# url-kaist/Quatro

Measured on NVIDIA H100. Metric: registrations/sec (64-ring pair), higher is better.
Workload: dtype f32 (front end, match, graph filter) / f64 (graph boundary, GNC, COTE)

## Files before the change

include/quatro_b200.h:

```cpp
#ifndef QUATRO_B200_H_
#define QUATRO_B200_H_

#include <stdint.h>

#ifdef __cplusplus
extern "C" {
#endif

#define QB200_VERSION 100

typedef enum qb200_status {
  QB200_OK = 0,
  QB200_DEGENERATE_CLIQUE = 1,
  QB200_DEGENERATE_INPUT = 2,
  QB200_CAPACITY_EXCEEDED = 3,
  QB200_ERR_BAD_ARG = -1,
  QB200_ERR_NO_DEVICE = -2,
  QB200_ERR_CUDA = -3,
  QB200_ERR_UNSUPPORTED = -4,
  QB200_ERR_VOXEL_OVERFLOW = -5
} qb200_status;

enum { QB200_FLAG_CLIQUE_TRUNCATED = 1  };
#define QB200_DEFAULT_CLIQUE_NODE_LIMIT 262144
// ... 154 lines not shown
                                const qb200_params* p, qb200_result* res);

int qb200_match_and_pack(qb200_handle* h, const float* src4, int32_t n_src, const float* tgt4,
                         int32_t n_tgt, const qb200_params* p, int32_t* corr, float* src_matched4,
                         float* tgt_matched4, int32_t cap, int32_t* n_corr);

typedef struct qb200_corr_set {
  const float* a;
  const float* b;
  int32_t L;
  int32_t reserved;
} qb200_corr_set;
int qb200_solve_batch(qb200_handle* h, const qb200_corr_set* sets, int32_t n_sets, const qb200_params* p,
                      qb200_mem_kind kind, qb200_result* results);

typedef struct qb200_pair_lists {
  int32_t cap_per_pair;
  int32_t kind;
  int32_t* corr;
  float* src_matched4;
  float* tgt_matched4;
  int32_t* clique;
  int32_t* final_inliers;
  uint8_t* rot_inlier_mask;
  uint8_t* trans_inlier_mask;
} qb200_pair_lists;
enum { QB200_FLAG_LISTS_TRUNCATED = 2  };

int qb200_solve_batch_ex(qb200_handle* h, const qb200_corr_set* sets, int32_t n_sets, const qb200_params* p, qb200_mem_kind kind,
                         qb200_result* results, const qb200_pair_lists* lists);

int qb200_register_batch_enqueue(qb200_handle* h, const qb200_pair* pairs, int32_t n_pairs, const qb200_params* p, qb200_mem_kind kind,
                                 qb200_result* results);
int qb200_register_batch_flush(qb200_handle* h);
int qb200_register_batch_enqueue_ex(qb200_handle* h, const qb200_pair* pairs, int32_t n_pairs, const qb200_params* p,
                                    qb200_mem_kind kind, qb200_result* results, const qb200_pair_lists* lists);

int qb200_register_pair(qb200_handle* h, const float* src4, int32_t n_src, const float* tgt4,
                        int32_t n_tgt, const qb200_params* p, qb200_result* res);

int qb200_register_batch(qb200_handle* h, const qb200_pair* pairs, int32_t n_pairs,
                         const qb200_params* p, qb200_mem_kind kind, qb200_result* results);
int qb200_register_batch_ex(qb200_handle* h, const qb200_pair* pairs, int32_t n_pairs, const qb200_params* p, qb200_mem_kind kind,
                            qb200_result* results, const qb200_pair_lists* lists);

typedef struct qb200_slot_pair { int32_t src_slot, tgt_slot; } qb200_slot_pair;
int qb200_cache_reserve(qb200_handle* h, int32_t n_slots);
int qb200_cache_scans(qb200_handle* h, const float* const* scans4, const int32_t* n_points, const int32_t* slot_ids, int32_t n_scans,
                      const qb200_params* p, qb200_mem_kind kind);
int qb200_register_cached(qb200_handle* h, const qb200_slot_pair* pairs, int32_t n_pairs, const qb200_params* p, qb200_result* results);
int qb200_register_cached_ex(qb200_handle* h, const qb200_slot_pair* pairs, int32_t n_pairs, const qb200_params* p,
                             qb200_result* results, const qb200_pair_lists* lists);
int qb200_cache_copy(qb200_handle* h, int32_t from_slot, int32_t to_slot);
int qb200_cache_read(qb200_handle* h, int32_t slot, float* vox4, float* normals4, float* desc33, int32_t cap, int32_t* n);

#define QB200_UNIQUE_ID_BYTES 128
int qb200_comm_init_all(qb200_handle** handles, int32_t n_dev);
int qb200_register_batch_sharded(qb200_handle** handles, int32_t n_dev, const qb200_pair* pairs, int32_t n_pairs,
                                 const qb200_params* p, qb200_mem_kind kind, qb200_result* results);
int qb200_comm_unique_id(void* id128);
int qb200_comm_init_rank(qb200_handle* h, int32_t world, int32_t rank, const void* id128);
int qb200_register_batch_rank(qb200_handle* h, const qb200_pair* local_pairs, int32_t n_local, const qb200_params* p,
                              qb200_mem_kind kind, qb200_result* all_results, int32_t defer);
int qb200_comm_wait(qb200_handle* h);
int qb200_bind_numa(qb200_handle* h);

int qb200_get_last_clique(qb200_handle* h, int32_t* idx, int32_t cap, int32_t* n);
int qb200_get_last_final_inliers(qb200_handle* h, int32_t* idx, int32_t cap, int32_t* n);
int qb200_get_last_correspondences(qb200_handle* h, int32_t* corr, float* src_matched4,
                                   float* tgt_matched4, int32_t cap, int32_t* n);

int qb200_get_last_features(qb200_handle* h, int32_t which, float* normals4, float* desc33, int32_t cap, int32_t* n);

int qb200_get_stage_ms(qb200_handle* h, float* ms, int32_t n);

int qb200_get_kernel_ms(qb200_handle* h, float* ms, int32_t* launches, int32_t n);

int qb200_debug_tc_distances(qb200_handle* h, const float* a33, int32_t na, const float* b33, int32_t nb, float* out);


int qb200_debug_match_stats(qb200_handle* h, uint64_t* out4, int32_t reset);
int qb200_debug_nn_tables(qb200_handle* h, uint64_t* rowbest, int32_t cap_rows, uint64_t* colbest, int32_t cap_cols);
int qb200_debug_tc_profile(qb200_handle* h, uint64_t* out24, int32_t reset);
int qb200_debug_tc_footprint(qb200_handle* h, int32_t* out5);

int qb200_debug_match_verify(qb200_handle* h, uint64_t* out2, int32_t reset);

#ifdef __cplusplus
}
#endif
#endif
```

quatro_b200/capi.py:

```python
from __future__ import annotations

import ctypes as C
from typing import Optional, Sequence

import numpy as np

from . import _build

PMC_EXACT, PMC_HEU, KCORE_HEU, INLIER_NONE = 0, 1, 2, 3
FLAG_CLIQUE_TRUNCATED = 1
FLAG_LISTS_TRUNCATED = 2
COTE_MEDIAN, COTE_WEIGHTED_MEAN = 0, 1
MEM_HOST, MEM_DEVICE = 0, 1

STATUS_NAMES = {0: "OK", 1: "DEGENERATE_CLIQUE", 2: "DEGENERATE_INPUT", 3: "CAPACITY_EXCEEDED", -1: "ERR_BAD_ARG",
                -2: "ERR_NO_DEVICE", -3: "ERR_CUDA", -4: "ERR_UNSUPPORTED", -5: "ERR_VOXEL_OVERFLOW"}


class Params(C.Structure):
    _fields_ = [
        ("voxel_size", C.c_float), ("normal_radius", C.c_float), ("fpfh_radius", C.c_float), ("grid_cell", C.c_float),
        ("tuple_scale", C.c_float), ("use_crosscheck", C.c_int32), ("use_tuple_test", C.c_int32),
        ("tuple_trials_per_corr", C.c_int32), ("skip_flagged", C.c_int32), ("reserved0", C.c_int32),
        ("seed", C.c_uint64),
# ... 98 lines not shown

    def trimmed(self, records: np.ndarray) -> list:
        out = []
        for i, r in enumerate(records):
            d = {}
            for name, a in self.arrays.items():
                m = 0 if r["status"] == 3 else min(int(r[LIST_LAYOUT[name][2]]), self.cap)
                d[name] = a[i, :m].copy() if self.kind == MEM_HOST else a[i, :m]
            out.append(d)
        return out


RESULT_DTYPE = np.dtype([
    ("valid", "<i4"), ("status", "<i4"), ("n_src_vox", "<i4"), ("n_tgt_vox", "<i4"), ("n_mutual", "<i4"),
    ("n_corr", "<i4"), ("max_core", "<i4"), ("clique_size", "<i4"), ("gnc_iters", "<i4"), ("n_rot_inliers", "<i4"),
    ("n_final_inliers", "<i4"), ("flags", "<i4"), ("n_edges", "<i8"), ("cost", "<f8"), ("T", "<f8", (16,)),
])
assert RESULT_DTYPE.itemsize == C.sizeof(Result)


class QuatroB200Error(RuntimeError):
    def __init__(self, code: int, where: str, detail: str = ""):
        self.code = code
        super().__init__(f"{where}: {STATUS_NAMES.get(code, code)} {detail}")


_LIB: Optional[C.CDLL] = None


def _f32(a, cols=None) -> np.ndarray:
    a = np.ascontiguousarray(a, dtype=np.float32)
    if cols is not None:
        assert a.ndim == 2 and a.shape[1] == cols, (a.shape, cols)
    return a


def _ptr(a: Optional[np.ndarray]):
    return None if a is None else a.ctypes.data_as(C.c_void_p)


def load_library(build: bool = True) -> C.CDLL:
    global _LIB
    if _LIB is not None:
        return _LIB
    path = _build.build_cuda() if build else _build.CUDA_LIB
    lib = C.CDLL(str(path))
    vp, i32, i64, f32, f64 = C.c_void_p, C.c_int32, C.c_int64, C.c_float, C.c_double
    P = C.POINTER
    sig = {
        "qb200_default_params": (None, [P(Params)]),
        "qb200_default_config": (None, [P(Config)]),
        "qb200_version": (i32, []),
        "qb200_create": (i32, [P(Config), P(vp)]),
        "qb200_destroy": (None, [vp]),
        "qb200_set_stream": (i32, [vp, vp]),
        "qb200_last_error": (C.c_char_p, [vp]),
        "qb200_launch_count": (i64, [vp]),
        "qb200_voxelize": (i32, [vp, vp, i32, f32, i32, vp, i32, P(i32)]),
        "qb200_default_patchwork_params": (None, [P(PatchworkParams)]),
        "qb200_default_segment_params": (None, [P(SegmentParams)]),
        "qb200_segment_cloud": (i32, [vp, vp, i32, P(SegmentParams), vp, P(i32), vp, P(i32)]),
        "qb200_patchwork": (i32, [vp, vp, i32, P(PatchworkParams), vp, P(i32), vp, P(i32)]),
        "qb200_compute_fpfh": (i32, [vp, vp, i32, f32, f32, f32, vp, vp]),
        "qb200_match": (i32, [vp, vp, i32, vp, vp, i32, vp, P(Params), vp, i32, P(i32), P(i32)]),
        "qb200_build_graph": (i32, [vp, vp, vp, i32, f64, f64, vp, i32, vp, P(i64)]),
        "qb200_max_clique": (i32, [vp, vp, i32, i32, i32, f64, vp, P(i32), vp, vp, P(i32)]),
        "qb200_max_clique_ex": (i32, [vp, vp, i32, i32, i32, f64, i64, vp, P(i32), vp, vp, P(i32), P(i32)]),
        "qb200_solve_pose": (i32, [vp, vp, vp, i32, vp, i32, P(Params), P(Result), vp, vp]),
        "qb200_solve_correspondences": (i32, [vp, vp, vp, i32, P(Params), P(Result)]),
        "qb200_match_and_pack": (i32, [vp, vp, i32, vp, i32, P(Params), vp, vp, vp, i32, P(i32)]),
        "qb200_register_pair": (i32, [vp, vp, i32, vp, i32, P(Params), P(Result)]),
        "qb200_register_batch": (i32, [vp, P(Pair), i32, P(Params), i32, vp]),
        "qb200_get_last_clique": (i32, [vp, vp, i32, P(i32)]),
        "qb200_get_last_final_inliers": (i32, [vp, vp, i32, P(i32)]),
        "qb200_get_last_correspondences": (i32, [vp, vp, vp, vp, i32, P(i32)]),
        "qb200_get_stage_ms": (i32, [vp, vp, i32]),
        "qb200_get_kernel_ms": (i32, [vp, vp, vp, i32]),
        "qb200_debug_tc_distances": (i32, [vp, vp, i32, vp, i32, vp]),
        "qb200_debug_match_stats": (i32, [vp, vp, i32]),
        "qb200_debug_nn_tables": (i32, [vp, vp, i32, vp, i32]),
        "qb200_register_batch_enqueue": (i32, [vp, vp, i32, vp, i32, vp]),
        "qb200_register_batch_flush": (i32, [vp]),
        "qb200_debug_tc_profile": (i32, [vp, vp, i32]),
        "qb200_debug_tc_footprint": (i32, [vp, vp]),
        "qb200_solve_batch": (i32, [vp, vp, i32, vp, i32, vp]),
        "qb200_comm_init_all": (i32, [P(vp), i32]),
        "qb200_register_batch_sharded": (i32, [P(vp), i32, P(Pair), i32, P(Params), i32, vp]),
        "qb200_comm_unique_id": (i32, [vp]),
        "qb200_comm_init_rank": (i32, [vp, i32, i32, vp]),
        "qb200_register_batch_rank": (i32, [vp, P(Pair), i32, P(Params), i32, vp, i32]),
        "qb200_comm_wait": (i32, [vp]),
        "qb200_bind_numa": (i32, [vp]),
        "qb200_debug_match_verify": (i32, [vp, vp, i32]),
        "qb200_get_last_features": (i32, [vp, i32, vp, vp, i32, P(i32)]),
        "qb200_cache_reserve": (i32, [vp, i32]),
        "qb200_cache_scans": (i32, [vp, P(vp), P(i32), P(i32), i32, P(Params), i32]),
        "qb200_register_cached": (i32, [vp, vp, i32, P(Params), vp]),
        "qb200_cache_copy": (i32, [vp, i32, i32]),
        "qb200_cache_read": (i32, [vp, i32, vp, vp, vp, i32, P(i32)]),
        "qb200_register_batch_ex": (i32, [vp, vp, i32, P(Params), i32, vp, P(PairLists)]),
        "qb200_register_batch_enqueue_ex": (i32, [vp, vp, i32, P(Params), i32, vp, P(PairLists)]),
        "qb200_register_cached_ex": (i32, [vp, vp, i32, P(Params), vp, P(PairLists)]),
        "qb200_solve_batch_ex": (i32, [vp, vp, i32, P(Params), i32, vp, P(PairLists)]),
    }
    for name, (res, args) in sig.items():
        fn = getattr(lib, name)
        fn.restype = res
        fn.argtypes = args
    _LIB = lib
    return lib


EXPORTED_SYMBOLS = [
    "qb200_default_params", "qb200_default_config", "qb200_version", "qb200_create", "qb200_destroy",
    "qb200_set_stream", "qb200_last_error", "qb200_launch_count", "qb200_voxelize", "qb200_compute_fpfh",
    "qb200_default_patchwork_params", "qb200_patchwork", "qb200_default_segment_params", "qb200_segment_cloud", "qb200_match", "qb200_build_graph", "qb200_max_clique", "qb200_max_clique_ex", "qb200_solve_pose", "qb200_solve_correspondences",
    "qb200_match_and_pack", "qb200_register_pair", "qb200_register_batch", "qb200_get_last_clique",
    "qb200_get_last_final_inliers", "qb200_get_last_correspondences", "qb200_get_stage_ms", "qb200_get_kernel_ms",
    "qb200_debug_tc_distances",
    "qb200_debug_match_stats",
    "qb200_debug_nn_tables",
    "qb200_register_batch_enqueue",
    "qb200_register_batch_flush",
    "qb200_debug_tc_profile",
    "qb200_debug_tc_footprint",
    "qb200_solve_batch",
    "qb200_comm_init_all", "qb200_register_batch_sharded", "qb200_comm_unique_id", "qb200_comm_init_rank",
    "qb200_register_batch_rank", "qb200_comm_wait", "qb200_bind_numa",
    "qb200_debug_match_verify", "qb200_get_last_features", "qb200_cache_reserve", "qb200_cache_scans", "qb200_register_cached", "qb200_cache_copy", "qb200_cache_read",
    "qb200_register_batch_ex", "qb200_register_batch_enqueue_ex", "qb200_register_cached_ex", "qb200_solve_batch_ex",
]


def default_params() -> Params:
    p = Params()
    p.voxel_size, p.normal_radius, p.fpfh_radius, p.grid_cell = 0.3, 0.5, 0.75, 0.0
    p.tuple_scale, p.use_crosscheck, p.use_tuple_test, p.tuple_trials_per_corr = 0.95, 1, 1, 100
    p.skip_flagged, p.seed = 1, 0x5EED
    p.noise_bound, p.cbar2, p.rot_noise_bound, p.cote_noise_bound = 0.3, 1.0, 0.0, 0.3
    p.rotation_gnc_factor, p.rotation_cost_threshold, p.kcore_heuristic_threshold = 1.4, 0.00011, 0.5
    p.rotation_max_iterations, p.inlier_selection_mode, p.cote_mode = 50, PMC_HEU, COTE_MEDIAN
    p.using_rot_inliers_when_estimating_cote, p.use_pre_estimated_RyRx = 0, 0
    for i in range(9):
        p.RyRx[i] = 1.0 if i in (0, 4, 8) else 0.0
    return p


def comm_init_all(handles: Sequence["Handle"]):
    arr = (C.c_void_p * len(handles))(*[h.h for h in handles])
    st = load_library().qb200_comm_init_all(arr, len(handles))
    if st != 0:
        raise QuatroB200Error(st, "qb200_comm_init_all")


def register_batch_sharded(handles: Sequence["Handle"], pairs: Sequence, params: "Params", kind: int = 0) -> np.ndarray:
    n = len(pairs)
    arr = (Pair * n)()
    keep = []
    for i, pr in enumerate(pairs):
        if kind == MEM_HOST:
            s, t = _f32(pr[0], 4), _f32(pr[1], 4)
            keep.append((s, t))
            arr[i].src, arr[i].n_src, arr[i].tgt, arr[i].n_tgt = s.ctypes.data, len(s), t.ctypes.data, len(t)
        else:
            arr[i].src, arr[i].n_src, arr[i].tgt, arr[i].n_tgt = pr[0], pr[1], pr[2], pr[3]
    out = np.zeros(n, RESULT_DTYPE)
    hs = (C.c_void_p * len(handles))(*[h.h for h in handles])
    st = load_library().qb200_register_batch_sharded(hs, len(handles), arr, n, C.byref(params), kind, _ptr(out))
    if st != 0:
        raise QuatroB200Error(st, "qb200_register_batch_sharded " + handles[0].last_error())
    return out


def default_patchwork_params() -> PatchworkParams:
    p = PatchworkParams()
    load_library().qb200_default_patchwork_params(C.byref(p))
    return p


def default_segment_params() -> SegmentParams:
    p = SegmentParams()
    load_library().qb200_default_segment_params(C.byref(p))
    return p


def default_config() -> Config:
    c = Config()
    c.device, c.max_batch_slots, c.max_raw_points, c.max_voxel_points, c.max_corr = 0, 64, 131072, 16384, 4096
    return c


class Handle:

    def __init__(self, config: Optional[Config] = None, **kw):
        self.lib = load_library()
        cfg = config or default_config()
        for k, v in kw.items():
            setattr(cfg, k, v)
        self.cfg = cfg
        h = C.c_void_p()
        st = self.lib.qb200_create(C.byref(cfg), C.byref(h))
        if st != 0:
            raise QuatroB200Error(st, "qb200_create")
        self.h = h

    def close(self):
        if getattr(self, "h", None):
# ... 237 lines not shown
        out = np.zeros(len(sp), RESULT_DTYPE)
        self._check(self.lib.qb200_register_cached(self.h, _ptr(sp), len(sp), C.byref(params), _ptr(out)), "qb200_register_cached")
        return out

    def cache_copy(self, from_slot: int, to_slot: int):
        self._check(self.lib.qb200_cache_copy(self.h, from_slot, to_slot), "qb200_cache_copy")

    def cache_read(self, slot: int, cap: Optional[int] = None):
        cap = cap or self.cfg.max_voxel_points
        vox, nrm, desc = np.zeros((cap, 4), np.float32), np.zeros((cap, 4), np.float32), np.zeros((cap, 33), np.float32)
        n = C.c_int32(0)
        self._check(self.lib.qb200_cache_read(self.h, slot, _ptr(vox), _ptr(nrm), _ptr(desc), cap, C.byref(n)), "qb200_cache_read")
        m = min(n.value, cap)
        return vox[:m].copy(), nrm[:m].copy(), desc[:m].copy()

    @staticmethod
    def comm_unique_id() -> bytes:
        buf = C.create_string_buffer(128)
        st = load_library().qb200_comm_unique_id(buf)
        if st != 0:
            raise QuatroB200Error(st, "qb200_comm_unique_id")
        return buf.raw

    def comm_init_rank(self, world: int, rank: int, unique_id: bytes):
        buf = C.create_string_buffer(unique_id, 128)
        self._check(self.lib.qb200_comm_init_rank(self.h, world, rank, buf), "qb200_comm_init_rank")
        self.world, self.rank = world, rank

    def register_batch_rank_raw(self, pair_array, n_local: int, params: Params, kind: int, out_all: np.ndarray, defer: bool = False):
        return self._check(self.lib.qb200_register_batch_rank(self.h, pair_array, n_local, C.byref(params), kind, _ptr(out_all), int(defer)),
                           "qb200_register_batch_rank")

    def bind_numa(self) -> int:
        return int(self.lib.qb200_bind_numa(self.h))

    def comm_wait(self):
        return self._check(self.lib.qb200_comm_wait(self.h), "qb200_comm_wait")

    def register_batch_raw(self, pair_array, n: int, params: Params, kind: int, out: np.ndarray):
        return self._check(self.lib.qb200_register_batch(self.h, pair_array, n, C.byref(params), kind, _ptr(out)), "qb200_register_batch")

    def register_batch_enqueue_raw(self, pair_array, n: int, params: Params, kind: int, out: np.ndarray):
        return self._check(self.lib.qb200_register_batch_enqueue(self.h, pair_array, n, C.byref(params), kind, _ptr(out)), "qb200_register_batch_enqueue")

    def register_batch_flush(self):
        return self._check(self.lib.qb200_register_batch_flush(self.h), "qb200_register_batch_flush")

    def last_clique(self, cap: int = 1 << 16):
        idx = np.zeros(cap, np.int32)
        n = C.c_int32(0)
        self._check(self.lib.qb200_get_last_clique(self.h, _ptr(idx), cap, C.byref(n)), "qb200_get_last_clique")
        return idx[: n.value].copy()

    def last_final_inliers(self, cap: int = 1 << 16):
        idx = np.zeros(cap, np.int32)
        n = C.c_int32(0)
        self._check(self.lib.qb200_get_last_final_inliers(self.h, _ptr(idx), cap, C.byref(n)), "qb200_get_last_final_inliers")
        return idx[: n.value].copy()

    def last_correspondences(self, cap: int = 1 << 16):
        corr = np.zeros((cap, 2), np.int32)
        sm = np.zeros((cap, 4), np.float32)
        tm = np.zeros((cap, 4), np.float32)
        n = C.c_int32(0)
        self._check(self.lib.qb200_get_last_correspondences(self.h, _ptr(corr), _ptr(sm), _ptr(tm), cap, C.byref(n)),
                    "qb200_get_last_correspondences")
        return corr[: n.value].copy(), sm[: n.value].copy(), tm[: n.value].copy()

    def debug_match_stats(self, reset: bool = True) -> dict:
        out = np.zeros(4, np.uint64)
        self._check(self.lib.qb200_debug_match_stats(self.h, _ptr(out), int(reset)), "qb200_debug_match_stats")
        return {"exact_evals": int(out[0]), "tiles": int(out[1]), "warmups": int(out[2]), "aborted_stripes": int(out[3])}

    def debug_nn_tables(self, n_src: int, n_tgt: int):
        rb, cb = np.full(n_src, ~np.uint64(0)), np.full(n_tgt, ~np.uint64(0))
        self._check(self.lib.qb200_debug_nn_tables(self.h, _ptr(rb), n_src, _ptr(cb), n_tgt), "qb200_debug_nn_tables")
        return rb, cb

    def debug_tc_profile(self, reset: bool = True) -> np.ndarray:
        out = np.zeros(24, np.uint64)
        self._check(self.lib.qb200_debug_tc_profile(self.h, _ptr(out), int(reset)), "qb200_debug_tc_profile")
        return out

    def debug_tc_footprint(self) -> dict:
        out = np.zeros(5, np.int32)
        self._check(self.lib.qb200_debug_tc_footprint(self.h, _ptr(out)), "qb200_debug_tc_footprint")
        return {"threads": int(out[0]), "dyn_smem": int(out[1]), "static_smem": int(out[2]), "regs": int(out[3]),
                "ctas_per_sm": int(out[4])}

    def debug_match_verify(self, reset: bool = True) -> dict:
        out = np.zeros(2, np.uint64)
        self._check(self.lib.qb200_debug_match_verify(self.h, _ptr(out), int(reset)), "qb200_debug_match_verify")
        return {"compared": int(out[0]), "mismatches": int(out[1])}

    def debug_tc_distances(self, a33, b33) -> np.ndarray:
        a33, b33 = _f32(a33, 33), _f32(b33, 33)
        out = np.zeros((128, 128), np.float32)
        self._check(self.lib.qb200_debug_tc_distances(self.h, _ptr(a33), len(a33), _ptr(b33), len(b33), _ptr(out)), "qb200_debug_tc_distances")
        return out[: len(a33), : len(b33)].copy()

    def kernel_ms(self):
        ms = np.zeros(2, np.float32)
        calls = np.zeros(2, np.int32)
        self.lib.qb200_get_kernel_ms(self.h, _ptr(ms), _ptr(calls), 2)
        return ms, calls

    def stage_ms(self) -> np.ndarray:
        ms = np.zeros(8, np.float32)
        self.lib.qb200_get_stage_ms(self.h, _ptr(ms), 8)
        return ms
```

quatro_b200/csrc/clique.cu:

```cuda
#include "handle.cuh"

namespace qb {

__device__ __forceinline__ int warp_max(int v) { return __reduce_max_sync(0xffffffffu, v); }
__device__ __forceinline__ int warp_sum(int v) { return __reduce_add_sync(0xffffffffu, v); }

__device__ void warp_bucket_sort(const unsigned short* __restrict__ key, int n, int maxkey, int* __restrict__ bin,
                                 unsigned short* __restrict__ pos, unsigned short* __restrict__ vert) {
  const int lane = lane_id();
  for (int d = lane; d <= maxkey + 1; d += 32) bin[d] = 0;
  __syncwarp();
  for (int v = lane; v < n; v += 32) atomicAdd(&bin[key[v]], 1);
  __syncwarp();
  int carry = 0;
  for (int base = 0; base <= maxkey + 1; base += 32) {
    const int d = base + lane;
    const int c = d <= maxkey + 1 ? bin[d] : 0;
    int tot;
    const int ex = warp_excl_scan(c, &tot);
    if (d <= maxkey + 1) bin[d] = carry + ex;
    carry += tot;
  }
  __syncwarp();
  for (int base = 0; base < n; base += 32) {
    const int v = base + lane;
    const bool act = v < n;
    const int d = act ? key[v] : -1 - lane;
    const unsigned peers = __match_any_sync(0xffffffffu, d);
    const int rank = __popc(peers & ((1u << lane) - 1));
    const int b = act ? bin[d] : 0;
    __syncwarp();
    if (act) {
      pos[v] = (unsigned short)(b + rank);
      vert[b + rank] = (unsigned short)v;
      if (rank == 0) bin[d] = b + __popc(peers);
    }
    __syncwarp();
  }
  for (int base = ((maxkey + 1) / 32) * 32; base >= 0; base -= 32) {
    const int d = base + lane;
    int prev = 0;
    if (d >= 1 && d <= maxkey + 1) prev = bin[d - 1];
    __syncwarp();
    if (d >= 1 && d <= maxkey + 1) bin[d] = prev;
    __syncwarp();
  }
  if (lane == 0) bin[0] = 0;
  __syncwarp();
}

constexpr int kRing = 16;

__device__ __forceinline__ void cp_async4(void* smem_dst, const void* gsrc) {
  const unsigned d = (unsigned)__cvta_generic_to_shared(smem_dst);
  asm volatile("cp.async.ca.shared.global [%0], [%1], 4;" ::"r"(d), "l"(gsrc) : "memory");
}
__device__ __forceinline__ void cp_async_commit() { asm volatile("cp.async.commit_group;" ::: "memory"); }
template <int N>
__device__ __forceinline__ void cp_async_wait() { asm volatile("cp.async.wait_group %0;" ::"n"(N) : "memory"); }

constexpr int kKcWarps = 4;

__device__ __forceinline__ void kcore_apply_moves(const unsigned short* __restrict__ nbl, int cnt, int dv, int* __restrict__ bin,
                                                  unsigned short* __restrict__ deg, unsigned short* __restrict__ pos,
                                                  unsigned short* __restrict__ vert, unsigned short* __restrict__ mrk,
                                                  uint32_t* __restrict__ above_own, uint32_t* __restrict__ add_next, bool classes) {
  const int lane = lane_id();
  const unsigned lt = (1u << lane) - 1u;
  for (int c0 = 0; c0 < cnt; c0 += 32) {
    const int e = c0 + lane;
    const bool act = e < cnt;
    const int u = act ? nbl[e] : 0;
    const int du = act ? deg[u] : -1 - lane;
    const unsigned grp = __match_any_sync(0xffffffffu, du);
    const int rank = __popc(grp & lt), m = __popc(grp);
    int b0 = 0, pu = 0;
    if (act) {
      b0 = bin[du];
      pu = pos[u];
      mrk[u] = (unsigned short)(rank + 1);
    }
    __syncwarp();
    int y = -1;
    if (act && pu >= b0 + m) {
      int curk = rank;
      for (;;) {
        y = vert[b0 + curk];
        const int r = mrk[y];
        if (r == 0) break;
        curk = r - 1;
      }
    }
    __syncwarp();
    if (act) {
      vert[b0 + rank] = (unsigned short)u; pos[u] = (unsigned short)(b0 + rank);
      if (y >= 0) { vert[pu] = (unsigned short)y; pos[y] = (unsigned short)pu; }
      mrk[u] = 0;
      deg[u] = (unsigned short)(du - 1);
      const uint32_t bit = 1u << (u & 31);
      if (classes) {
        atomicAnd(&above_own[u >> 5], ~bit);
        if (du - 1 > dv) atomicOr(&add_next[u >> 5], bit);
      } else if (du - 1 == dv) {
        atomicAnd(&above_own[u >> 5], ~bit);
      }
      if (rank == 0) bin[du] = b0 + m;
    }
    __syncwarp();
  }
}

template <int WPL>
__device__ __forceinline__ int kcore_expand(const uint32_t (&w)[WPL], int w0, unsigned short* __restrict__ nbl) {
  int c = 0;
#pragma unroll
  for (int k = 0; k < WPL; ++k) c += __popc(w[k]);
  int cnt;
  int off = warp_excl_scan(c, &cnt);
  if (cnt != 0) {
#pragma unroll
    for (int k = 0; k < WPL; ++k) {
      uint32_t x = w[k];
      const int basebit = (w0 + k) * 32;
      while (x) {
        const int b = __ffs(x) - 1;
        x &= x - 1;
        nbl[off++] = (unsigned short)(basebit + b);
      }
    }
  }
  return cnt;
}

template <int WPL, bool kWs>
__global__ void __maxnreg__(168) kcore_kernel(const uint32_t* __restrict__ adj, const int* __restrict__ deg_in,
                                                              const int* __restrict__ n_corr, int Lc, int W, int Ls, int row_words,
                                                              unsigned char* __restrict__ ws, int* __restrict__ kcore,
                                                              int* __restrict__ korder, int* __restrict__ rank_of, int* __restrict__ by_rank,
                                                              int* __restrict__ kbin, int* __restrict__ max_core_out) {
  constexpr int NW = kKcWarps, AW = 32 * WPL;
  extern __shared__ __align__(16) unsigned char smem_raw[];
  __shared__ int ring_tag[kRing];

  const int pair = blockIdx.x, tid = threadIdx.x, lane = tid & 31, warp = tid >> 5;
  const int L = n_corr[pair];
  if ((L > Ls) != kWs) return;
  constexpr bool in_smem = !kWs;
  const int Lv = in_smem ? Ls : Lc;
  int* bin = in_smem ? reinterpret_cast<int*>(smem_raw)
                     : reinterpret_cast<int*>(ws + (size_t)pair * kcore_ws_bytes(Lc));
  uint32_t* above = in_smem ? reinterpret_cast<uint32_t*>(bin + Ls + 2)
                            : reinterpret_cast<uint32_t*>(smem_raw);
  uint32_t* add = above + NW * AW;
  uint32_t* rows = add + 2 * NW * AW;
  unsigned short* deg = in_smem ? reinterpret_cast<unsigned short*>(rows + row_words) : reinterpret_cast<unsigned short*>(bin + Lc + 2);
  unsigned short* pos = deg + Lv;
  unsigned short* vert = pos + Lv;
  unsigned short* mrk = vert + Lv;
  unsigned short* nbl_all = mrk + Lv;
  int* __restrict__ kc = kcore + (size_t)pair * (Lc + 2);
  int* __restrict__ ko = korder + (size_t)pair * (Lc + 2);
  int* __restrict__ ro = rank_of + (size_t)pair * (Lc + 2);
  int* __restrict__ br = by_rank + (size_t)pair * (Lc + 2);
  int* __restrict__ kb = kbin + (size_t)pair * (Lc + 2);
  if (L <= 0) {
    if (tid == 0) max_core_out[pair] = 0;
    return;
  }
  const uint32_t* __restrict__ G = adj + (size_t)pair * Lc * W;
  const int nbw = (L + 31) >> 5;
  const int nwl = (nbw + 31) >> 5;
  const bool cached = in_smem && (long long)L * nbw <= (long long)row_words;
  const int rs = in_smem ? Ls / 32 : W;
  const int w0 = lane * nwl;
  unsigned short* nbl = nbl_all + (size_t)warp * Lv;

  int md = 0;
  for (int v = tid; v < L; v += NW * 32) {
    const int d = deg_in[(size_t)pair * Lc + v];
    deg[v] = (unsigned short)d;
    mrk[v] = 0;
    md = max(md, d);
  }
  if (cached)
    for (int idx = tid; idx < L * nbw; idx += NW * 32) rows[idx] = G[(size_t)(idx / nbw) * W + (idx % nbw)];
  for (int wd = tid; wd < 3 * NW * AW; wd += NW * 32) above[wd] = 0u;
  __shared__ int s_md[NW];
  md = warp_max(md);
  if (lane == 0) s_md[warp] = md;
  __syncthreads();
  md = max(max(s_md[0], s_md[1]), max(s_md[2], s_md[3]));
  if (warp == 0) warp_bucket_sort(deg, L, md, bin, pos, vert);
  __syncthreads();
  for (int v = tid; v < L; v += NW * 32) {
    const int c = cached ? 0 : (int)deg[v] % NW;
    atomicOr(&above[c * AW + (v >> 5)], 1u << (v & 31));
  }
  __syncthreads();

  int cur = -1;
  if (cached) {
    if (warp != 0) return;
    for (int i = 0; i < L; ++i) {
      const int v = vert[i];
      const int dv = deg[v];
      if (dv > cur) {
        const int end = bin[dv + 1];
        for (int p = i + lane; p < end; p += 32) {
          const int x = vert[p];
          atomicAnd(&above[x >> 5], ~(1u << (x & 31)));
        }
        cur = dv;
        __syncwarp();
      }
      uint32_t w[WPL];
#pragma unroll
      for (int k = 0; k < WPL; ++k) w[k] = (k < nwl && w0 + k < nbw) ? (rows[v * nbw + w0 + k] & above[w0 + k]) : 0u;
      const int cnt = kcore_expand<WPL>(w, w0, nbl);
      if (cnt == 0) continue;
      __syncwarp();
      kcore_apply_moves(nbl, cnt, dv, bin, deg, pos, vert, mrk, above, above, false);
    }
  } else {
    uint32_t* above_w = above + warp * AW;
    const int lower = (warp + NW - 1) % NW;
    auto fetch = [&](int p) {
      if (p < L) {
        const int x = vert[p], sl = p % kRing;
        if (lane == 0) ring_tag[sl] = x;
#pragma unroll
        for (int k = 0; k < WPL; ++k)
          if (k < nwl && w0 + k < nbw) cp_async4(rows + sl * rs + w0 + k, G + (size_t)x * W + w0 + k);
      }
      cp_async_commit();
    };
    if (warp == 0) {
      for (int p = 0; p < kRing - 1; ++p) fetch(p);
      cp_async_wait<kRing - 2>();
    }
    __syncthreads();
    for (int i = 0; i < L; ++i) {
      const int v = vert[i];
      const int dv = deg[v];
      const int par = i & 1;
      if (warp == 0) fetch(i + kRing - 1);
      uint32_t* add_in = add + ((par ^ 1) * NW + warp) * AW;
      uint32_t w[WPL];
      const int sl = i % kRing;
      const bool hit = ring_tag[sl] == v;
#pragma unroll
      for (int k = 0; k < WPL; ++k) {
        w[k] = 0u;
        if (k < nwl && w0 + k < nbw) {
          const uint32_t a = add_in[w0 + k];
          if (a) { above_w[w0 + k] |= a; add_in[w0 + k] = 0u; }
          w[k] = hit ? rows[sl * rs + w0 + k] : G[(size_t)v * W + w0 + k];
        }
      }
      __syncwarp();
      if (dv > cur) {
        if (dv % NW == warp) {
          const int end = bin[dv + 1];
          for (int p = i + lane; p < end; p += 32) {
            const int x = vert[p];
            atomicAnd(&above_w[x >> 5], ~(1u << (x & 31)));
          }
          __syncwarp();
        }
        cur = dv;
      }
#pragma unroll
      for (int k = 0; k < WPL; ++k) w[k] = (k < nwl && w0 + k < nbw) ? (w[k] & above_w[w0 + k]) : 0u;
      const int cnt = kcore_expand<WPL>(w, w0, nbl);
      if (cnt != 0) {
        __syncwarp();
        kcore_apply_moves(nbl, cnt, dv, bin, deg, pos, vert, mrk, above_w, add + (par * NW + lower) * AW, true);
      }
      if (warp == 0) cp_async_wait<kRing - 2>();
      __syncthreads();
    }
    if (warp == 0) cp_async_wait<0>();
    if (warp != 0) return;
  }
  __syncwarp();
  const int max_core = deg[vert[L - 1]];
  for (int v = lane; v < L; v += 32) {
    kc[v] = (int)deg[v] + 1;
    ko[v] = vert[v];
  }
  if (lane == 0) max_core_out[pair] = max_core;
  __syncwarp();
  warp_bucket_sort(deg, L, max_core, bin, pos, vert);
  for (int v = lane; v < L; v += 32) {
    ro[v] = pos[v];
    br[v] = vert[v];
  }
  for (int d = lane; d <= max_core + 1; d += 32) kb[d] = bin[d];
}

__global__ void __launch_bounds__(256) permute_adj_kernel(const uint32_t* __restrict__ adj, const int* __restrict__ n_corr, int Lc, int W,
                                                          const int* __restrict__ rank_of, uint32_t* __restrict__ adjp) {
  extern __shared__ uint32_t rows[];
  const int pair = blockIdx.y;
  const int L = n_corr[pair];
  const int wib = threadIdx.x >> 5, lane = lane_id();
// ... 280 lines not shown
    const int begin = lb[depth];
    const uint32_t e = LP[begin + n_here - 1];
    __syncwarp();
    if (lane == 0) ln[depth] = n_here - 1;
    const int v = (int)(e & 0xFFFFu), col = (int)(e >> 16);
    if (depth + col <= best) {
      if (lane == 0) ln[depth] = 0;
      __syncwarp();
      continue;
    }
    if (lane == 0) C[depth] = (unsigned short)v;
    uint32_t* __restrict__ Pl = SP + (size_t)depth * W;
    int cnt = 0;
#pragma unroll
    for (int k = 0; k < WPL; ++k) {
      const int wi = lane + 32 * k;
      uint32_t x = 0u;
      if (wi < nbw) {
        const uint32_t pw = Pl[wi];
        x = pw & rows[(size_t)v * stride + wi];
        if (wi == (v >> 5)) Pl[wi] = pw & ~(1u << (v & 31));
      }
      P[k] = x;
      cnt += __popc(x);
    }
    cnt = __reduce_add_sync(0xffffffffu, cnt);
    __syncwarp();
    if (cnt == 0) {
      if (depth + 1 > best) {
        best = depth + 1;
        improved = true;
        for (int t = lane; t <= depth; t += 32) out[t] = br[C[t]];
        __syncwarp();
        if (best >= ub) break;
      }
      continue;
    }
    if (depth + 1 + cnt <= best) continue;
    if (++nodes > node_limit || depth + 1 >= kExactDepth) { truncated = true; break; }
    const int nbegin = begin + n_here - 1;
    uint32_t* __restrict__ Pn = SP + (size_t)(depth + 1) * W;
#pragma unroll
    for (int k = 0; k < WPL; ++k) {
      const int wi = lane + 32 * k;
      if (wi < nbw) Pn[wi] = P[k];
    }
    const int nl = exact_colour_sort<WPL>(rows, stride, nbw, P, best - (depth + 1), LP + nbegin, kExactPool - nbegin);
    if (nl < 0) { truncated = true; break; }
    if (lane == 0) { lb[depth + 1] = nbegin; ln[depth + 1] = nl; }
    __syncwarp();
    ++depth;
  }
  __syncwarp();
  if (improved) {
    for (int t = lane; t < best; t += 32) {
      const int x = out[t];
      int r = 0;
      for (int u = 0; u < best; ++u) r += out[u] < x ? 1 : 0;
      lb[r] = x;
    }
    __syncwarp();
    for (int t = lane; t < best; t += 32) out[t] = lb[t];
    if (lane == 0) n_clique[pair] = best;
  }
  if (lane == 0 && truncated) flags[pair] |= QB200_FLAG_CLIQUE_TRUNCATED;
}

constexpr size_t kKcoreSmemBudget = 144 * 1024;

template <int WPL>
static int launch_kcore(Lane* h, int n_pairs) {
  const int Lc = h->Lc, W = h->W;
  const int Ls = Lc < kKcoreSmemVerts ? Lc : kKcoreSmemVerts, Ws = Ls / 32;
  const size_t bits = (size_t)3 * kKcWarps * 32 * WPL * sizeof(uint32_t);
  const size_t fixed = (size_t)(Ls + 2) * sizeof(int) + bits + (size_t)(4 + kKcWarps) * Ls * sizeof(unsigned short);
  size_t row_words = fixed + 8 * 1024 < kKcoreSmemBudget ? (kKcoreSmemBudget - fixed) / 4 : 0;
  if (row_words < (size_t)kRing * Ws) row_words = (size_t)kRing * Ws;
  if (row_words > (size_t)Ls * Ws) row_words = (size_t)Ls * Ws;
  const size_t smem = fixed + row_words * 4;
  if (Ls < Lc && smem - bits < (size_t)kRing * W * 4) {
    h->fail(__FILE__, __LINE__, "k-core prefetch ring does not fit");
    return QB200_ERR_CUDA;
  }
  QB_CUDA_TRY(h, ensure_dyn_smem(h->device, (const void*)kcore_kernel<WPL, false>, smem));
  kcore_kernel<WPL, false><<<n_pairs, kKcWarps * 32, smem, h->stream>>>(h->adj, h->deg, h->ctr.n_corr, Lc, W, Ls, (int)row_words, h->kcore_ws,
                                                                        h->kcore, h->korder, h->rank_of, h->by_rank, h->kbin, h->ctr.max_core);
  if (Ls < Lc) {
    QB_CUDA_TRY(h, ensure_dyn_smem(h->device, (const void*)kcore_kernel<WPL, true>, smem));
    kcore_kernel<WPL, true><<<n_pairs, kKcWarps * 32, smem, h->stream>>>(h->adj, h->deg, h->ctr.n_corr, Lc, W, Ls, (int)row_words, h->kcore_ws,
                                                                         h->kcore, h->korder, h->rank_of, h->by_rank, h->kbin, h->ctr.max_core);
    h->launches++;
  }
  return QB200_OK;
}

static int ensure_exact_scratch(Lane* h) {
  if (h->ex_stack) return QB200_OK;
  const size_t S = h->S < kExactChunk ? h->S : kExactChunk;
  DeviceMem<uint32_t> stack, pool;
  DeviceMem<int> lvl;
  DeviceMem<unsigned short> cur;
  QB_CUDA_TRY(h, stack.alloc(S * kExactDepth * (size_t)h->W));
  QB_CUDA_TRY(h, pool.alloc(S * (size_t)kExactPool));
  QB_CUDA_TRY(h, lvl.alloc(S * 2 * (size_t)kExactDepth));
  QB_CUDA_TRY(h, cur.alloc(S * (size_t)kExactDepth));
  h->ex_stack = std::move(stack);
  h->ex_pool = std::move(pool);
  h->ex_lvl = std::move(lvl);
  h->ex_cur = std::move(cur);
  return QB200_OK;
}

template <int WPL>
static int launch_exact(Lane* h, int n_pairs, long long node_limit, int cache_words) {
  QB_CUDA_TRY(h, ensure_dyn_smem(h->device, (const void*)clique_exact_kernel<WPL>, (size_t)cache_words * 4));
  const int chunk = h->S < kExactChunk ? h->S : kExactChunk;
  for (int base = 0; base < n_pairs; base += chunk) {
    const int np = n_pairs - base < chunk ? n_pairs - base : chunk;
    clique_exact_kernel<WPL><<<np, 32, (size_t)cache_words * 4, h->stream>>>(
        h->adjp, h->ctr.n_corr, h->Lc, h->W, h->by_rank, h->rank_of, h->kbin, h->ctr.max_core, node_limit, cache_words, base, h->ex_stack,
        h->ex_pool, h->ex_lvl, h->ex_lvl + (size_t)chunk * kExactDepth, h->ex_cur, h->clique, h->ctr.n_clique, h->ctr.flags);
    h->launches++;
  }
  return QB200_OK;
}

int launch_clique(Lane* h, int n_pairs, int mode, double kcore_thr, long long node_limit) {
  if (n_pairs <= 0) return QB200_OK;
  const int Lc = h->Lc, W = h->W;
  const int Ls = Lc < kKcoreSmemVerts ? Lc : kKcoreSmemVerts;
  const int cache_words = 14336;
  const size_t sm_clique = (size_t)kCliqueWarps * Ls * sizeof(unsigned short) + (size_t)W * sizeof(uint32_t) + (size_t)cache_words * 4;
  int rc;
  QB_CUDA_TRY(h, ensure_dyn_smem(h->device, (const void*)clique_cta_kernel, sm_clique));
  if (mode == QB200_PMC_EXACT && (rc = ensure_exact_scratch(h))) return rc;
  if (W <= 32) rc = launch_kcore<1>(h, n_pairs);
  else if (W <= 64) rc = launch_kcore<2>(h, n_pairs);
  else if (W <= 128) rc = launch_kcore<4>(h, n_pairs);
  else if (W <= 256) rc = launch_kcore<8>(h, n_pairs);
  else if (W <= 512) rc = launch_kcore<16>(h, n_pairs);
  else rc = launch_kcore<32>(h, n_pairs);
  if (rc) return rc;
  const dim3 gp((Lc + 7) / 8, n_pairs);
  permute_adj_kernel<<<gp, 256, 8 * W * sizeof(uint32_t), h->stream>>>(h->adj, h->ctr.n_corr, Lc, W, h->rank_of, h->adjp);
  clique_cta_kernel<<<n_pairs, kCliqueWarps * 32, sm_clique, h->stream>>>(h->adjp, h->ctr.n_corr, Lc, W, Ls, h->chain_ws, h->kcore, h->korder,
                                                                          h->rank_of, h->by_rank, h->kbin, h->ctr.max_core,
                                                                          mode == QB200_PMC_EXACT ? QB200_PMC_HEU : mode, kcore_thr, cache_words,
                                                                          h->clique, h->ctr.n_clique);
  h->launches += 3;
  if (mode == QB200_PMC_EXACT) {
    const long long lim = node_limit > 0 ? node_limit : (long long)QB200_DEFAULT_CLIQUE_NODE_LIMIT;
    if (W <= 32) rc = launch_exact<1>(h, n_pairs, lim, cache_words);
    else if (W <= 64) rc = launch_exact<2>(h, n_pairs, lim, cache_words);
    else if (W <= 128) rc = launch_exact<4>(h, n_pairs, lim, cache_words);
    else if (W <= 256) rc = launch_exact<8>(h, n_pairs, lim, cache_words);
    else if (W <= 512) rc = launch_exact<16>(h, n_pairs, lim, cache_words);
    else rc = launch_exact<32>(h, n_pairs, lim, cache_words);
    if (rc) return rc;
  }
  QB_CUDA_TRY(h, cudaGetLastError());
  return QB200_OK;
}

}
```

quatro_b200/csrc/stages.cu:

```cuda
#include <math.h>
#include <vector>

#include "handle.cuh"

using namespace qb;

namespace {

int read_counters(Lane* L) {
  QB_CUDA_TRY(L, cudaMemcpyAsync(L->hctr_block, L->ctr_block, L->ctr_ints * sizeof(int), cudaMemcpyDeviceToHost, L->stream));
  return QB200_OK;
}

int write_counter(Lane* L, int* host_slot, int value) {
  *host_slot = value;
  QB_CUDA_TRY(L, cudaMemcpyAsync(L->ctr_block + (host_slot - L->hctr_block), host_slot, sizeof(int), cudaMemcpyHostToDevice, L->stream));
  return QB200_OK;
}

struct MirrorHold {
  Lane* L; bool idle = false;
  ~MirrorHold() { if (!idle) cudaStreamSynchronize(L->stream); }
  cudaError_t sync() { idle = true; return cudaStreamSynchronize(L->stream); }
};
// ... 232 lines not shown
  if (rc) return rc;
  if (L > 0) QB_CUDA_TRY(h, cudaMemcpyAsync(ln->ma, a4, (size_t)L * sizeof(float4), cudaMemcpyHostToDevice, ln->stream));
  if (L > 0) QB_CUDA_TRY(h, cudaMemcpyAsync(ln->mb, b4, (size_t)L * sizeof(float4), cudaMemcpyHostToDevice, ln->stream));
  MirrorHold hold{ln};
  if ((rc = write_counter(ln, ln->hctr.n_corr, L)) || (rc = run_solver(ln, 1, resolve_params(h, *p), 0))) return rc;
  QB_CUDA_TRY(h, cudaMemcpyAsync(ln->h_results, ln->d_results, sizeof(qb200_result), cudaMemcpyDeviceToHost, ln->stream));
  QB_CUDA_TRY(h, hold.sync());
  *res = ln->h_results[0];
  set_last(h, *res);
  return res->status;
}

int qb200_get_last_clique(qb200_handle* h, int32_t* idx, int32_t cap, int32_t* n) {
  if (int rc = enter(h)) return rc;
  if (!n || cap < 0) return QB200_ERR_BAD_ARG;
  Lane* L = h->lane[0].get();
  *n = h->last_n_clique;
  const int m = *n < cap ? *n : cap;
  if (m > 0 && idx) {
    QB_CUDA_TRY(h, cudaMemcpyAsync(idx, L->clique, (size_t)m * sizeof(int), cudaMemcpyDeviceToHost, L->stream));
    QB_CUDA_TRY(h, cudaStreamSynchronize(L->stream));
  }
  return *n > cap ? QB200_CAPACITY_EXCEEDED : QB200_OK;
}

int qb200_get_last_final_inliers(qb200_handle* h, int32_t* idx, int32_t cap, int32_t* n) {
  if (int rc = enter(h)) return rc;
  if (!n || cap < 0) return QB200_ERR_BAD_ARG;
  Lane* L = h->lane[0].get();
  *n = h->last_n_final;
  const int m = *n < cap ? *n : cap;
  if (m > 0 && idx) {
    QB_CUDA_TRY(h, cudaMemcpyAsync(idx, L->final_inl, (size_t)m * sizeof(int), cudaMemcpyDeviceToHost, L->stream));
    QB_CUDA_TRY(h, cudaStreamSynchronize(L->stream));
  }
  return *n > cap ? QB200_CAPACITY_EXCEEDED : QB200_OK;
}

int qb200_get_last_correspondences(qb200_handle* h, int32_t* corr, float* src_matched4, float* tgt_matched4, int32_t cap, int32_t* n) {
  if (int rc = enter(h)) return rc;
  if (!n || cap < 0) return QB200_ERR_BAD_ARG;
  Lane* L = h->lane[0].get();
  *n = h->last_n_corr;
  const int m = *n < cap ? *n : cap;
  if (m > 0) {
    std::vector<int> s(m), t(m);
    QB_CUDA_TRY(h, cudaMemcpyAsync(s.data(), L->corr_src, (size_t)m * sizeof(int), cudaMemcpyDeviceToHost, L->stream));
    QB_CUDA_TRY(h, cudaMemcpyAsync(t.data(), L->corr_tgt, (size_t)m * sizeof(int), cudaMemcpyDeviceToHost, L->stream));
    if (src_matched4) QB_CUDA_TRY(h, cudaMemcpyAsync(src_matched4, L->ma, (size_t)m * sizeof(float4), cudaMemcpyDeviceToHost, L->stream));
    if (tgt_matched4) QB_CUDA_TRY(h, cudaMemcpyAsync(tgt_matched4, L->mb, (size_t)m * sizeof(float4), cudaMemcpyDeviceToHost, L->stream));
    QB_CUDA_TRY(h, cudaStreamSynchronize(L->stream));
    if (corr)
      for (int i = 0; i < m; ++i) { corr[2 * i] = s[i]; corr[2 * i + 1] = t[i]; }
  }
  return *n > cap ? QB200_CAPACITY_EXCEEDED : QB200_OK;
}

int qb200_get_last_features(qb200_handle* h, int32_t which, float* normals4, float* desc33, int32_t cap, int32_t* n_out) {
  if (int rc = enter(h)) return rc;
  if (!n_out || which < 0 || which > 1 || cap < 0) return QB200_ERR_BAD_ARG;
  Lane* L = h->lane[0].get();
  if (int rc = read_counters(L)) return rc;
  QB_CUDA_TRY(h, cudaStreamSynchronize(L->stream));
  const int n = L->hctr.n_vox[which];
  *n_out = n;
  const int m = n < cap ? n : cap;
  if (m > 0) {
    if (normals4) QB_CUDA_TRY(h, cudaMemcpyAsync(normals4, L->normals + (size_t)which * L->V, (size_t)m * sizeof(float4), cudaMemcpyDeviceToHost, L->stream));
    if (desc33) {
      if (int rc = launch_desc_to_aos(L, which, m, L->aos_scratch)) return rc;
      QB_CUDA_TRY(h, cudaMemcpyAsync(desc33, L->aos_scratch, (size_t)m * kDescDim * sizeof(float), cudaMemcpyDeviceToHost, L->stream));
    }
    QB_CUDA_TRY(h, cudaStreamSynchronize(L->stream));
  }
  return n > cap ? QB200_CAPACITY_EXCEEDED : QB200_OK;
}

int qb200_debug_match_verify(qb200_handle* h, uint64_t* out2, int32_t reset) { return read_tc_stats(h, 4, 2, out2, reset); }

int qb200_debug_tc_profile(qb200_handle* h, uint64_t* out24, int32_t reset) { return read_tc_stats(h, 8, 24, out24, reset); }

int qb200_debug_match_stats(qb200_handle* h, uint64_t* out4, int32_t reset) { return read_tc_stats(h, 0, 4, out4, reset); }

int qb200_debug_nn_tables(qb200_handle* h, uint64_t* rowbest, int32_t cap_rows, uint64_t* colbest, int32_t cap_cols) {
  if (int rc = enter(h)) return rc;
  if (cap_rows < 0 || cap_cols < 0) return QB200_ERR_BAD_ARG;
  Lane* L = h->lane[0].get();
  QB_CUDA_TRY(h, cudaStreamSynchronize(L->stream));
  const int nr = cap_rows < h->last_match_n[0] ? cap_rows : h->last_match_n[0];
  const int nc = cap_cols < h->last_match_n[1] ? cap_cols : h->last_match_n[1];
  if (rowbest && nr > 0) QB_CUDA_TRY(h, cudaMemcpy(rowbest, L->rowbest, (size_t)nr * 8, cudaMemcpyDeviceToHost));
  if (colbest && nc > 0) QB_CUDA_TRY(h, cudaMemcpy(colbest, L->colbest, (size_t)nc * 8, cudaMemcpyDeviceToHost));
  return QB200_OK;
}

int qb200_debug_tc_footprint(qb200_handle* h, int32_t* out5) {
  if (!h || !out5) return QB200_ERR_BAD_ARG;
  cudaSetDevice(h->cfg.device);
  return tc_footprint(h->lane[0].get(), out5);
}

int qb200_debug_tc_distances(qb200_handle* h, const float* a33, int32_t na, const float* b33, int32_t nb, float* out) {
  if (int rc = enter(h)) return rc;
  if (!a33 || !b33 || !out || na < 1 || nb < 1 || na > 128 || nb > 128) return QB200_ERR_BAD_ARG;
  Lane* L = h->lane[0].get();
  int rc = wave_reset(L, 2);
  if (rc) return rc;
  float* scratch = L->aos_scratch;
  QB_CUDA_TRY(h, cudaMemcpyAsync(scratch, a33, (size_t)na * kDescDim * sizeof(float), cudaMemcpyHostToDevice, L->stream));
  QB_CUDA_TRY(h, cudaMemcpyAsync(scratch + (size_t)128 * kDescDim, b33, (size_t)nb * kDescDim * sizeof(float), cudaMemcpyHostToDevice, L->stream));
  MirrorHold hold{L};
  if ((rc = write_counter(L, L->hctr.n_vox, na)) || (rc = write_counter(L, L->hctr.n_vox + 1, nb))) return rc;
  if ((rc = launch_desc_from_aos(L, 0, na, scratch)) || (rc = launch_desc_from_aos(L, 1, nb, scratch + (size_t)128 * kDescDim))) return rc;
  float* d_out = L->spfh;
  QB_CUDA_TRY(h, cudaMemsetAsync(d_out, 0, 128 * 128 * sizeof(float), L->stream));
  if ((rc = launch_tc_debug_tile(L, d_out))) return rc;
  QB_CUDA_TRY(h, cudaMemcpyAsync(out, d_out, 128 * 128 * sizeof(float), cudaMemcpyDeviceToHost, L->stream));
  QB_CUDA_TRY(h, hold.sync());
  return QB200_OK;
}

}
```

Measured before the change: 12870.

## Speculatively expand next k-core vertex on a helper warp in sparse graphs

The k-core peeling kernel gets a two-warp 'solo' path used when the graph is cached or its average degree is at most 128. A second warp speculatively computes the neighbor list of the next vertex in peel order into a double buffer, and prefetches rows several steps ahead into L1. The main warp reuses that list when the guess matches, so the serial peel loop no longer waits on row loads and expansion. It also filters neighbors by degree before the match_any grouping in apply_moves, and adds an optional profiling counter for speculation hits. The cost is a 64-thread named barrier every iteration, and the speculative list can go stale because it is built before the current vertex's moves are applied.

Measured after the change: 12850 (median of 6 runs). No clear change (-0.1%).

```diff
diff --git a/include/quatro_b200.h b/include/quatro_b200.h
--- a/include/quatro_b200.h
+++ b/include/quatro_b200.h
@@ -260,6 +260,7 @@
 int qb200_debug_match_stats(qb200_handle* h, uint64_t* out4, int32_t reset);
 int qb200_debug_nn_tables(qb200_handle* h, uint64_t* rowbest, int32_t cap_rows, uint64_t* colbest, int32_t cap_cols);
 int qb200_debug_tc_profile(qb200_handle* h, uint64_t* out24, int32_t reset);
+int qb200_debug_kcore_spec(qb200_handle* h, uint64_t* out2, int32_t reset);
 int qb200_debug_tc_footprint(qb200_handle* h, int32_t* out5);
 
 int qb200_debug_match_verify(qb200_handle* h, uint64_t* out2, int32_t reset);
diff --git a/quatro_b200/capi.py b/quatro_b200/capi.py
--- a/quatro_b200/capi.py
+++ b/quatro_b200/capi.py
@@ -204,6 +204,7 @@
         "qb200_register_batch_enqueue": (i32, [vp, vp, i32, vp, i32, vp]),
         "qb200_register_batch_flush": (i32, [vp]),
         "qb200_debug_tc_profile": (i32, [vp, vp, i32]),
+        "qb200_debug_kcore_spec": (i32, [vp, vp, i32]),
         "qb200_debug_tc_footprint": (i32, [vp, vp]),
         "qb200_solve_batch": (i32, [vp, vp, i32, vp, i32, vp]),
         "qb200_comm_init_all": (i32, [P(vp), i32]),
@@ -245,6 +246,7 @@
     "qb200_register_batch_enqueue",
     "qb200_register_batch_flush",
     "qb200_debug_tc_profile",
+    "qb200_debug_kcore_spec",
     "qb200_debug_tc_footprint",
     "qb200_solve_batch",
     "qb200_comm_init_all", "qb200_register_batch_sharded", "qb200_comm_unique_id", "qb200_comm_init_rank",
@@ -648,6 +650,11 @@
         self._check(self.lib.qb200_debug_tc_profile(self.h, _ptr(out), int(reset)), "qb200_debug_tc_profile")
         return out
 
+    def debug_kcore_spec(self, reset: bool = True) -> np.ndarray:
+        out = np.zeros(2, np.uint64)
+        self._check(self.lib.qb200_debug_kcore_spec(self.h, _ptr(out), int(reset)), "qb200_debug_kcore_spec")
+        return out
+
     def debug_tc_footprint(self) -> dict:
         out = np.zeros(5, np.int32)
         self._check(self.lib.qb200_debug_tc_footprint(self.h, _ptr(out)), "qb200_debug_tc_footprint")
diff --git a/quatro_b200/csrc/clique.cu b/quatro_b200/csrc/clique.cu
--- a/quatro_b200/csrc/clique.cu
+++ b/quatro_b200/csrc/clique.cu
@@ -60,6 +60,7 @@
 __device__ __forceinline__ void cp_async_wait() { asm volatile("cp.async.wait_group %0;" ::"n"(N) : "memory"); }
 
 constexpr int kKcWarps = 4;
+constexpr int kRowAhead = 8;
 
 __device__ __forceinline__ void kcore_apply_moves(const unsigned short* __restrict__ nbl, int cnt, int dv, int* __restrict__ bin,
                                                   unsigned short* __restrict__ deg, unsigned short* __restrict__ pos,
@@ -69,9 +70,10 @@
   const unsigned lt = (1u << lane) - 1u;
   for (int c0 = 0; c0 < cnt; c0 += 32) {
     const int e = c0 + lane;
-    const bool act = e < cnt;
-    const int u = act ? nbl[e] : 0;
-    const int du = act ? deg[u] : -1 - lane;
+    const int u = e < cnt ? nbl[e] : 0;
+    const int d = e < cnt ? deg[u] : -1;
+    const bool act = d > dv;
+    const int du = act ? d : -1 - lane;
     const unsigned grp = __match_any_sync(0xffffffffu, du);
     const int rank = __popc(grp & lt), m = __popc(grp);
     int b0 = 0, pu = 0;
@@ -132,12 +134,13 @@
   return cnt;
 }
 
-template <int WPL, bool kWs>
+template <int WPL, bool kWs, bool kProf = false>
 __global__ void __maxnreg__(168) kcore_kernel(const uint32_t* __restrict__ adj, const int* __restrict__ deg_in,
                                                               const int* __restrict__ n_corr, int Lc, int W, int Ls, int row_words,
                                                               unsigned char* __restrict__ ws, int* __restrict__ kcore,
                                                               int* __restrict__ korder, int* __restrict__ rank_of, int* __restrict__ by_rank,
-                                                              int* __restrict__ kbin, int* __restrict__ max_core_out) {
+                                                              int* __restrict__ kbin, int* __restrict__ max_core_out,
+                                                              unsigned long long* __restrict__ stats) {
   constexpr int NW = kKcWarps, AW = 32 * WPL;
   extern __shared__ __align__(16) unsigned char smem_raw[];
   __shared__ int ring_tag[kRing];
@@ -175,52 +178,92 @@
   const int w0 = lane * nwl;
   unsigned short* nbl = nbl_all + (size_t)warp * Lv;
 
-  int md = 0;
+  int md = 0, sd = 0;
   for (int v = tid; v < L; v += NW * 32) {
     const int d = deg_in[(size_t)pair * Lc + v];
     deg[v] = (unsigned short)d;
     mrk[v] = 0;
     md = max(md, d);
+    sd += d;
   }
   if (cached)
     for (int idx = tid; idx < L * nbw; idx += NW * 32) rows[idx] = G[(size_t)(idx / nbw) * W + (idx % nbw)];
   for (int wd = tid; wd < 3 * NW * AW; wd += NW * 32) above[wd] = 0u;
-  __shared__ int s_md[NW];
+  __shared__ int s_md[NW], s_sd[NW];
   md = warp_max(md);
-  if (lane == 0) s_md[warp] = md;
+  sd = warp_sum(sd);
+  if (lane == 0) { s_md[warp] = md; s_sd[warp] = sd; }
   __syncthreads();
   md = max(max(s_md[0], s_md[1]), max(s_md[2], s_md[3]));
+  const bool solo = cached || (long long)s_sd[0] + s_sd[1] + s_sd[2] + s_sd[3] <= 128LL * L;
   if (warp == 0) warp_bucket_sort(deg, L, md, bin, pos, vert);
   __syncthreads();
   for (int v = tid; v < L; v += NW * 32) {
-    const int c = cached ? 0 : (int)deg[v] % NW;
+    const int c = solo ? 0 : (int)deg[v] % NW;
     atomicOr(&above[c * AW + (v >> 5)], 1u << (v & 31));
   }
   __syncthreads();
 
   int cur = -1;
-  if (cached) {
+  auto live_words = [&](int x, uint32_t (&w)[WPL]) {
+    if (cached) {
+#pragma unroll
+      for (int k = 0; k < WPL; ++k) w[k] = (k < nwl && w0 + k < nbw) ? (rows[x * nbw + w0 + k] & above[w0 + k]) : 0u;
+    } else {
+#pragma unroll
+      for (int k = 0; k < WPL; ++k) w[k] = (k < nwl && w0 + k < nbw) ? (__ldg(G + (size_t)x * W + w0 + k) & above[w0 + k]) : 0u;
+    }
+  };
+  if (solo) {
+    if (warp > 1) return;
+    __shared__ int s_guess[2], s_cnt[2];
+    if (tid < 2) s_guess[tid] = -1;
+    asm volatile("bar.sync 1, 64;" ::: "memory");
+    unsigned long long n_hit = 0, n_miss = 0;
+    for (int i = 0; i < L; ++i) {
+      const int b = i & 1;
+      if (warp == 0) {
+        unsigned short* lst = nbl_all + (size_t)b * Lv;
+        const int v = vert[i];
+        const int dv = deg[v];
+        if (dv > cur) {
+          const int end = bin[dv + 1];
+          for (int p = i + lane; p < end; p += 32) {
+            const int x = vert[p];
+            atomicAnd(&above[x >> 5], ~(1u << (x & 31)));
+          }
+          cur = dv;
+          __syncwarp();
+        }
+        int cnt;
+        if (s_guess[b] == v) {
+          cnt = s_cnt[b];
+          if (kProf) ++n_hit;
+        } else {
+          uint32_t w[WPL];
+          live_words(v, w);
+          cnt = kcore_expand<WPL>(w, w0, lst);
+          if (kProf && i > 0) ++n_miss;
+        }
+        if (cnt != 0) {
+          __syncwarp();
+          kcore_apply_moves(lst, cnt, dv, bin, deg, pos, vert, mrk, above, above, false);
+        }
+      } else if (i + 1 < L) {
+        if (!cached && i + kRowAhead < L && lane < nwl) {
+          const uint32_t* r = G + (size_t)vert[i + kRowAhead] * W + lane * 32;
+          asm volatile("prefetch.global.L1 [%0];" ::"l"(r));
+        }
+        const int g = vert[i + 1];
+        uint32_t w[WPL];
+        live_words(g, w);
+        const int cnt = kcore_expand<WPL>(w, w0, nbl_all + (size_t)(b ^ 1) * Lv);
+        if (lane == 0) { s_guess[b ^ 1] = g; s_cnt[b ^ 1] = cnt; }
+      }
+      asm volatile("bar.sync 1, 64;" ::: "memory");
+    }
     if (warp != 0) return;
-    for (int i = 0; i < L; ++i) {
-      const int v = vert[i];
-      const int dv = deg[v];
-      if (dv > cur) {
-        const int end = bin[dv + 1];
-        for (int p = i + lane; p < end; p += 32) {
-          const int x = vert[p];
-          atomicAnd(&above[x >> 5], ~(1u << (x & 31)));
-        }
-        cur = dv;
-        __syncwarp();
-      }
-      uint32_t w[WPL];
-#pragma unroll
-      for (int k = 0; k < WPL; ++k) w[k] = (k < nwl && w0 + k < nbw) ? (rows[v * nbw + w0 + k] & above[w0 + k]) : 0u;
-      const int cnt = kcore_expand<WPL>(w, w0, nbl);
-      if (cnt == 0) continue;
-      __syncwarp();
-      kcore_apply_moves(nbl, cnt, dv, bin, deg, pos, vert, mrk, above, above, false);
-    }
+    if (kProf && lane == 0) { atomicAdd(stats + 6, n_hit); atomicAdd(stats + 7, n_miss); }
   } else {
     uint32_t* above_w = above + warp * AW;
     const int lower = (warp + NW - 1) % NW;
@@ -667,13 +710,16 @@
     h->fail(__FILE__, __LINE__, "k-core prefetch ring does not fit");
     return QB200_ERR_CUDA;
   }
-  QB_CUDA_TRY(h, ensure_dyn_smem(h->device, (const void*)kcore_kernel<WPL, false>, smem));
-  kcore_kernel<WPL, false><<<n_pairs, kKcWarps * 32, smem, h->stream>>>(h->adj, h->deg, h->ctr.n_corr, Lc, W, Ls, (int)row_words, h->kcore_ws,
-                                                                        h->kcore, h->korder, h->rank_of, h->by_rank, h->kbin, h->ctr.max_core);
+  const bool prof = getenv("QB200_KCORE_PROF") && getenv("QB200_KCORE_PROF")[0] == '1';
+  const auto kshared = prof ? kcore_kernel<WPL, false, true> : kcore_kernel<WPL, false>;
+  QB_CUDA_TRY(h, ensure_dyn_smem(h->device, (const void*)kshared, smem));
+  kshared<<<n_pairs, kKcWarps * 32, smem, h->stream>>>(h->adj, h->deg, h->ctr.n_corr, Lc, W, Ls, (int)row_words, h->kcore_ws, h->kcore,
+                                                        h->korder, h->rank_of, h->by_rank, h->kbin, h->ctr.max_core, h->tc_stats);
   if (Ls < Lc) {
     QB_CUDA_TRY(h, ensure_dyn_smem(h->device, (const void*)kcore_kernel<WPL, true>, smem));
     kcore_kernel<WPL, true><<<n_pairs, kKcWarps * 32, smem, h->stream>>>(h->adj, h->deg, h->ctr.n_corr, Lc, W, Ls, (int)row_words, h->kcore_ws,
-                                                                         h->kcore, h->korder, h->rank_of, h->by_rank, h->kbin, h->ctr.max_core);
+                                                                         h->kcore, h->korder, h->rank_of, h->by_rank, h->kbin, h->ctr.max_core,
+                                                                         h->tc_stats);
     h->launches++;
   }
   return QB200_OK;
diff --git a/quatro_b200/csrc/stages.cu b/quatro_b200/csrc/stages.cu
--- a/quatro_b200/csrc/stages.cu
+++ b/quatro_b200/csrc/stages.cu
@@ -338,6 +338,8 @@
 
 int qb200_debug_match_stats(qb200_handle* h, uint64_t* out4, int32_t reset) { return read_tc_stats(h, 0, 4, out4, reset); }
 
+int qb200_debug_kcore_spec(qb200_handle* h, uint64_t* out2, int32_t reset) { return read_tc_stats(h, 6, 2, out2, reset); }
+
 int qb200_debug_nn_tables(qb200_handle* h, uint64_t* rowbest, int32_t cap_rows, uint64_t* colbest, int32_t cap_cols) {
   if (int rc = enter(h)) return rc;
   if (cap_rows < 0 || cap_cols < 0) return QB200_ERR_BAD_ARG;
```
